# agussomacal/ROMHighContrast

Hardware: AMD Instinct MI355X
Metric: snapshot_solves_per_sec (higher is better)
Workload: dtype f64

## Files before the change

### romhighcontrast_amd/csrc/rom_fem_dev.h

```cpp
#pragma once
#include "rom_mma.h"

struct FemDev {
  int nrb, ncb, N, n1, n1p, nr, nc, nGp, nGa, T, nslots, kblk, npre, nrhs, nexp, ncross, xb0;
  long long dim;
  const double* pool;
  const int* alist;
  const int* aoff;
  int tile_stream;
  const int* pairs;
  int npairs;
  const double* pool_acc;
  const int* wmeta;
  int wp0[5];
  int s1_t0, s1_nterm, s1_ndr;
  const int* s1_items;
  const int* s1_citems;
  const GenTerm* terms;
  const double* Bt;
  const double* P;
  const double* vec;
  const RhsTerm* rhs;
  const PreEdge* pre;
  const ExpEdge* exp;
  const int* xred;
  const int* scb;
  int spos0, nsc, sblk0;
  const DenseGroup* dgroups;
  const int* dweight;
  const int* ditem_group;
  const int* ditem_k;
  const double* dmat;
  int ndg, ndi;
  const CoefGroup* groups;
  const double* cm;
  const int* item_group;
  const int* item_k;
  const int* item_cf;
  const int* ctask;
  int nctask, ncf;
  double* gdots;
  int ncoef;
  const double* G;
  const double* Gs;
  const double* A0;
  const double* Qp;
  const int* kmax;
  const int* epos;
  double* yhat;
  const double* W;
  const double* g;
  const TileDesc* desc;
  const int* kptr;
  const int* kpair;
  const int* colptr;
  const int* colrow;
  const int* colti;
  const BlockSide* sides;
  int n_lr;
  const int* lr_blocks;
  const int* gen_blocks;
  const int* vmap;
  const int* scat;
  int nscat;
  double* L;
  double* invL;
  double* y;
  int* status;
};


FemDev make_dev(const rom_fem* f);

constexpr int COEF_MAX = 64;
#ifndef PAIR_RING_
#define PAIR_RING_ 8
#endif
constexpr int PAIR_RING = PAIR_RING_;
constexpr int S1_COEF_BYTES = 4 * COEF_MAX * 8, S1_WAVE_BYTES = (40 * 64 + 64 * 4 + 64 + 64 + 3 * 64 * 4) * 8;
constexpr int S1_ITEM_PASSES = 4;
constexpr int S1_DENSE_BYTES = 64 * 64 * 8;
constexpr int S1_LDS_BYTES = S1_COEF_BYTES + 4 * S1_WAVE_BYTES + S1_DENSE_BYTES;
constexpr int DENSE_GROUPS_MAX = 8;

__host__ __device__ inline int h0_row(int s, int i, int j, int N, int n1) {
  int ii, jj;
  switch (s) {
    case 0: ii = i; jj = j; break;
    case 1: ii = N - i; jj = j; break;
    case 2: ii = j; jj = i; break;
    default: ii = N - j; jj = i; break;
  }
  return (ii - 1) * n1 + (jj - 1);
}

__global__ void k_repack_table(const double* __restrict__ G, int ld, int nseg, int n1, int orient, double* __restrict__ Gs);
__global__ void k_build_A0(double* A0, const double* Qp, const double* rho, int n1, int n1p, int N);
__global__ void k_rhs(FemDev f, const double* __restrict__ a);
__global__ void k_coef(FemDev f, const double* __restrict__ a);
__global__ void k_expand(FemDev f, const double* __restrict__ a, int Mc, double* __restrict__ U, long long row0);
__global__ void k_back_pre(FemDev f, const double* __restrict__ a, int Mc);
template <int NS>
__global__ void k_diag_update(FemDev f, const double* __restrict__ a, int slot, int Mc);
__global__ void k_diag_factor(FemDev f, int slot, int j);
__global__ void k_solve1(FemDev f, const double* __restrict__ a, int Mc);
template <int NS>
__global__ void k_factor_panel(FemDev f, const double* __restrict__ a, int j, int Mc);
__global__ void k_backsolve(FemDev f);
__global__ void k_edge_transform(FemDev f, int Mc);
__global__ void k_extend(FemDev f, const double* __restrict__ a, int Mc, double* __restrict__ U, long long row0, const int* __restrict__ blocks, int pw_log2);
constexpr int X128_BLOCKS = 16;
// ... 65 lines not shown
```

### romhighcontrast_amd/csrc/rom_fem_kernels.hip

```cpp
#include "rom_fem_dev.h"

__global__ void k_build_A0(double* A0, const double* Qp, const double* rho, int n1, int n1p, int N) {
  size_t idx = blockIdx.x * size_t(blockDim.x) + threadIdx.x;
  size_t total = size_t(n1) * n1 * n1p;
  if (idx >= total) return;
  int m = int(idx % n1p);
  size_t ij = idx / n1p;
  int j = int(ij % n1) + 1, i = int(ij / n1) + 1;
  A0[idx] = (m < n1) ? Qp[size_t(j - 1) * n1p + m] * rho[size_t(m) * (N + 1) + i] : 0.0;
}

__global__ void k_repack_table(const double* __restrict__ G, int ld, int nseg, int n1, int orient, double* __restrict__ Gs) {
  const long long idx = blockIdx.x * (long long)blockDim.x + threadIdx.x;
  const long long hrows = (long long)n1 * n1;
  if (idx >= (long long)nseg * hrows * 8) return;
  const int kk = int(idx & 7);
  const long long rp = (idx >> 3) % hrows, seg = (idx >> 3) / hrows;
  const long long row = orient ? (rp % n1) * n1 + rp / n1 : rp;
  const int k = int(seg) * 8 + kk;
  Gs[idx] = k < ld ? G[row * ld + k] : 0.0;
}


__device__ inline double readlane_f64(double v, int lane) {
// ... 1333 lines not shown
  for (int v = t; v < f.nGa; v += 256) ym[v] = xs[v];
}

__global__ __launch_bounds__(256) void k_edge_transform(FemDev f, int Mc) {
  __shared__ __align__(16) double lds[STAGE_TOTAL];
  const WavePos wp;
  const int pos = f.epos[blockIdx.z];
  const int srow = stage_row(), sseg = stage_seg();
  const int mA = blockIdx.y * 64 + srow;
  const double* pA = mA < Mc ? f.y + size_t(mA) * f.nGp + pos + sseg : nullptr;
  const double* pB = f.Qp + size_t(blockIdx.x * 64 + srow) * f.n1p + sseg;
  Acc acc;
  acc_zero(acc);
  gemm_loop(
      f.n1p / BK, [&](int ch, double* v) { load4_aligned(pA ? pA + ch * BK : nullptr, v); },
      [&](int ch, double* v) { load4_aligned(pB + ch * BK, v); }, acc, lds, wp);
#pragma unroll
  for (int i = 0; i < 2; ++i)
#pragma unroll
    for (int g = 0; g < 4; ++g) {
      const int m = blockIdx.y * 64 + acc_row(wp, i, g);
      if (m >= Mc) continue;
#pragma unroll
      for (int jb = 0; jb < 2; ++jb)
        f.yhat[size_t(m) * f.nGp + pos + blockIdx.x * 64 + acc_col(wp, jb)] = acc.c[i][jb][g];
    }
}


__global__ __launch_bounds__(256) void k_extend(FemDev f, const double* __restrict__ a, int Mc,
                                                double* __restrict__ U, long long row0, const int* __restrict__ blocks,
                                                int pw_log2) {
  __shared__ __align__(16) double lds[STAGE_TOTAL];
  __shared__ double scs[64];
  double* stage = lds;
  const WavePos wp;
  const int b = blocks[blockIdx.z];
  const int p = b / f.ncb, q = b % f.ncb;
  const int n1 = f.n1, N = f.N;
  const BlockSide& sd = f.sides[b];
  const int srow = stage_row(), sseg = stage_seg();
  const int pw = 1 << pw_log2, ph = 64 >> pw_log2;
  const int npj = (n1 + pw - 1) >> pw_log2;
  const int pi = blockIdx.x / npj, pj = blockIdx.x % npj;
  const int i0 = ph * pi + 1, j0 = pw * pj + 1;
  const int i1 = min(i0 + ph - 1, n1), j1 = min(j0 + pw - 1, n1);

  const int mA = blockIdx.y * 64 + srow;
  const bool vA = mA < Mc;
  const int iB = i0 + (srow >> pw_log2), jB = j0 + (srow & (pw - 1));
  const bool vB = iB <= n1 && jB <= n1;

  int cend[4];
  const double* pAs[4];
  const double* pBs[4];
  int tot = 0;
#pragma unroll
  for (int s = 0; s < 4; ++s) {
    const ExtSide es = sd.s[s];
    int nch = 0;
    pAs[s] = pBs[s] = nullptr;
    if (es.mode != 0) {
      const int hrow = vB ? h0_row(s, iB, jB, N, n1) : 0;
      if (es.mode == 1) {
        const int dist = s == 0 ? i0 : s == 1 ? N - i1 : s == 2 ? j0 : N - j1;
        nch = f.kmax[dist] / BK;
        if (vA) pAs[s] = f.yhat + size_t(mA) * f.nGp + es.off + sseg;
        if (vB) pBs[s] = f.A0 + size_t(hrow) * f.n1p + sseg;
      } else {
        nch = es.nch;
        if (vA) pAs[s] = f.y + size_t(mA) * f.nGp + es.off + sseg;
        if (vB) pBs[s] = f.G + es.gtab + size_t(hrow) * (es.nch * BK) + sseg;
      }
    }
    tot += nch;
    cend[s] = tot;
  }
  if (threadIdx.x < 64) {
    const int m = blockIdx.y * 64 + threadIdx.x;
    scs[threadIdx.x] = m < Mc ? f.y[size_t(m) * f.nGp + f.sblk0 + b] : 0.0;
  }
  __syncthreads();
  Acc acc;
  acc_zero(acc);
  auto pick = [&](int ch, const double* const* ps) -> const double* {
    const int s = (ch >= cend[0]) + (ch >= cend[1]) + (ch >= cend[2]);
    const int lc = ch - (s == 0 ? 0 : s == 1 ? cend[0] : s == 2 ? cend[1] : cend[2]);
    const double* p = s == 0 ? ps[0] : s == 1 ? ps[1] : s == 2 ? ps[2] : ps[3];
    return p ? p + lc * BK : nullptr;
  };
  gemm_loop(
      tot, [&](int ch, double* v) { load4_aligned(pick(ch, pAs), v); },
      [&](int ch, double* v) { load4_aligned(pick(ch, pBs), v); }, acc, stage, wp);

  const bool odd = wp.lane & 1;
  const int cfirst = acc_col(wp, odd ? 1 : 0) - (odd ? 1 : 0);
  const int ii = i0 + (cfirst >> pw_log2) - 1, jj = j0 + (cfirst & (pw - 1)) - 1;
  const bool v0 = ii < n1 && jj < n1, v1 = ii < n1 && jj + 1 < n1;
  const long long gidx = (long long)(p * N + ii) * f.nc + (q * N + jj);
  double w_own[2];
#pragma unroll
  for (int jb = 0; jb < 2; ++jb) {
    const int cidx = acc_col(wp, jb);
    const int wi = i0 + (cidx >> pw_log2) - 1, wj = j0 + (cidx & (pw - 1)) - 1;
    w_own[jb] = (wi < n1 && wj < n1) ? f.W[wi * n1 + wj] : 0.0;
  }
#pragma unroll
  for (int i = 0; i < 2; ++i)
#pragma unroll
    for (int g = 0; g < 4; ++g) {
      const int m = blockIdx.y * 64 + acc_row(wp, i, g);
      const double sc = scs[acc_row(wp, i, g)];
      const double x0 = acc.c[i][0][g] + sc * w_own[0], x1 = acc.c[i][1][g] + sc * w_own[1];
      const double got = lane_swap1(odd ? x0 : x1);
      if (m >= Mc) continue;
      double* dst = U + (row0 + m) * f.dim + gidx;
      const double lo = odd ? got : x0, hi = odd ? x1 : got;
      if (v1) *reinterpret_cast<double2_u*>(dst) = double2_u{lo, hi};
      else if (v0) dst[0] = lo;
    }
}



constexpr int X128_SLOT = 4 * 128 * 64;

template <bool FLAT>
__global__ __launch_bounds__(512, 2) void k_extend128(FemDev f, X128Args xa, const double* __restrict__ a, int Mc,
                                                      double* __restrict__ U, long long row0, int with_expand,
                                                      int sys_fast) {
  __shared__ __align__(16) char lds_bytes[2 * X128_SLOT];
  __shared__ double scs[128];
  double* const lds = reinterpret_cast<double*>(lds_bytes);
  const int n1 = f.n1, N = f.N;
  const int nct = (n1 + 127) / 128;
  const int nvert = n1 * n1;
  const int ntile = FLAT ? (nvert + 127) / 128 : n1 * nct;
  int bx, by, ngy;
  if (sys_fast > 0) {
    bx = int(blockIdx.x) / sys_fast; by = int(blockIdx.x) % sys_fast; ngy = sys_fast;
  } else if (sys_fast < 0) {
    ngy = -sys_fast;
    const int unit = int(blockIdx.x) / (8 * ngy), r = int(blockIdx.x) % (8 * ngy);
    bx = unit * 8 + (r & 7); by = r >> 3;
  } else {
    bx = int(blockIdx.x); by = int(blockIdx.y); ngy = int(gridDim.y);
  }
  if (bx >= ntile + with_expand) return;
  if (bx >= ntile) {
    static_assert(STAGE_TOTAL * sizeof(double) <= 2 * X128_SLOT, "expansion staging must fit");
    const int nx = f.n1p / 64, ny = (Mc + 63) / 64;
    const int item = (bx - ntile) + with_expand * (by + ngy * blockIdx.z);
    if (threadIdx.x >= 256) return;
    if (item < nx * ny * (f.nexp + 1)) expand_tile(f, Mc, U, row0, lds, item % nx, (item / nx) % ny, item / (nx * ny));
    return;
  }
  const int bz = blockIdx.z;
  {
    const unsigned lin = __builtin_amdgcn_readfirstlane(blockIdx.x + gridDim.x * (blockIdx.y + gridDim.y * bz));
    if (lin >= 256u && lin < 512u)
      for (int i = 0; i < 2; ++i) __builtin_amdgcn_s_sleep(127);
  }
  const int b = xa.blocks[bz];
  const int p = b / f.ncb, q = b % f.ncb;
  const BlockSide sd = xa.sides[bz];
  const int iv = bx / nct + 1;
  const int jv0 = 128 * (bx % nct) + 1;
  const int vt0 = 128 * bx;
  const int lane = threadIdx.x & 63, w = __builtin_amdgcn_readfirstlane(threadIdx.x >> 6), wr = w >> 2, wc = w & 3;
  constexpr int NJ = 2;
  const int fr = lane & 15, kq = lane >> 4;
  double my_sc = 0.0;
  if (threadIdx.x < 128) {
    const int m = by * 128 + threadIdx.x;
    if (m < Mc) my_sc = f.y[size_t(m) * f.nGp + f.sblk0 + b];
  }
  double w_own[NJ];
#pragma unroll
  for (int j = 0; j < NJ; ++j) {
    if (FLAT) {
      const int v = vt0 + wc * (16 * NJ) + j * 16 + fr;
      w_own[j] = v < nvert ? f.W[v] : 0.0;
    } else {
      const int jj = jv0 + wc * (16 * NJ) + j * 16 + fr;
      w_own[j] = jj <= n1 ? f.W[(iv - 1) * n1 + (jj - 1)] : 0.0;
    }
  }
  const int cnt0 = sd.s[0].mode == 2 ? min(2 * sd.s[0].nch, (sd.s[0].r + 1 + 7) / 8) : 0;
  const int cnt1 = sd.s[1].mode == 2 ? min(2 * sd.s[1].nch, (sd.s[1].r + 1 + 7) / 8) : 0;
  const int cnt2 = sd.s[2].mode == 2 ? min(2 * sd.s[2].nch, (sd.s[2].r + 1 + 7) / 8) : 0;
  const int cnt3 = sd.s[3].mode == 2 ? min(2 * sd.s[3].nch, (sd.s[3].r + 1 + 7) / 8) : 0;
  const int nseg = cnt0 + cnt1 + cnt2 + cnt3;
  const int tot = (nseg + 1) / 2;
  const unsigned fx = unsigned((kq >> 1) ^ (fr >> 2));
  const unsigned fa0 = unsigned(fr * 64) + (fx << 4) + unsigned(kq & 1) * 8u;
  const unsigned fa1 = unsigned(fr * 64) + ((fx ^ 2u) << 4) + unsigned(kq & 1) * 8u;
#define X_FRAGS(SLOT_, KKI_, AF_, BF_)                                                                             \
  do {                                                                                                             \
    const char* pf_ = lds_bytes + (SLOT_) * X128_SLOT + (((KKI_)&1) ? fa1 : fa0);                                  \
    const char* pa_ = pf_ + ((KKI_) >> 1) * 8192 + wr * 4096;                                                      \
    const char* pb_ = pf_ + 16384 + ((KKI_) >> 1) * 8192 + wc * (1024 * NJ);                                       \
    _Pragma("unroll") for (int i_ = 0; i_ < 4; ++i_) AF_[i_] = *reinterpret_cast<const double*>(pa_ + i_ * 1024);  \
    _Pragma("unroll") for (int i_ = 0; i_ < NJ; ++i_) BF_[i_] = *reinterpret_cast<const double*>(pb_ + i_ * 1024); \
  } while (0)
  const unsigned lds0 = unsigned(size_t((__attribute__((address_space(3))) char*)lds_bytes));
  const unsigned du16 = unsigned(((lane & 3) ^ ((lane >> 4) & 3)) * 16);
  const unsigned ybytes_row = unsigned(f.nGp) * 8u;
  const int m0 = by * 128;
  unsigned voA[2];
  int vi[2], vj[2];
#pragma unroll
  for (int g = 0; g < 2; ++g) {
    const int rl = 32 * (w & 3) + 16 * g + (lane >> 2);
    voA[g] = unsigned(max(0, min(rl, Mc - 1 - m0))) * ybytes_row + du16;
    if (FLAT) {
      const int v = min(vt0 + rl, nvert - 1);
      vi[g] = v / n1 + 1;
      vj[g] = v % n1 + 1;
    } else {
      vi[g] = iv;
      vj[g] = min(jv0 + rl, n1);
    }
  }
  const char* const ybase = reinterpret_cast<const char*>(f.y) + size_t(min(m0, Mc - 1)) * ybytes_row;
  const char* const gsbase = reinterpret_cast<const char*>(f.Gs);
  const size_t seg_stride = size_t(n1) * n1 * 64;
  const char* const zbase = reinterpret_cast<const char*>(f.W + size_t(n1) * n1);
  const unsigned voZ = unsigned(lane) * 16u;
  int c_side = -1, c_left = 0, c_segs = nseg;
  const char* pA = zbase;
  const char* pB = zbase;
  unsigned voB[2] = {0, 0};
#define X_NEXT_SIDE()                                                                                              \
  do {                                                                                                             \
    do {                                                                                                           \
      ++c_side;                                                                                                    \
      c_left = c_side == 0 ? cnt0 : c_side == 1 ? cnt1 : c_side == 2 ? cnt2 : cnt3;                                \
    } while (c_left == 0 && c_side < 3);                                                                           \
    const int off_ = c_side == 0 ? sd.s[0].off : c_side == 1 ? sd.s[1].off : c_side == 2 ? sd.s[2].off : sd.s[3].off; \
    const int gseg_ = c_side == 0 ? sd.s[0].gseg : c_side == 1 ? sd.s[1].gseg : c_side == 2 ? sd.s[2].gseg : sd.s[3].gseg; \
     \
         \
    const int ci_ = c_side == 1 ? -n1 : n1, cj_ = c_side == 3 ? -1 : 1;                                             \
    const int k0_ = c_side == 1 ? n1 * n1 - 1 : c_side == 3 ? -n1 + n1 : -n1 - 1;                                   \
    pA = ybase + size_t(off_) * 8;                                                                                 \
    pB = gsbase + size_t(gseg_) * 8;                                                                               \
    voB[0] = unsigned(ci_ * vi[0] + cj_ * vj[0] + k0_) * 64u + du16;                                               \
    voB[1] = unsigned(ci_ * vi[1] + cj_ * vj[1] + k0_) * 64u + du16;                                               \
  } while (0)
#define X_DMA(LDS_, BASE_, VOFF_)                                                                                  \
  asm volatile("s_mov_b32 m0, %0\n\tglobal_load_lds_dwordx4 %1, %2" ::"s"(__builtin_amdgcn_readfirstlane(LDS_)),   \
               "v"(VOFF_), "s"(x128_uniform(BASE_))                                                                \
               : "memory", "m0")
#define X_ISSUE_HALF(SLOT_, H_, MINE_)                                                                             \
  do {                                                                                                             \
    const unsigned sb_ = lds0 + unsigned(SLOT_) * X128_SLOT + (H_) * 8192 + unsigned(w & 3) * 2048;                \
    if (c_segs > 0) {                                                                                              \
      if (MINE_) {                                                                                                 \
        X_DMA(sb_, pA, voA[0]);                                                                                    \
        X_DMA(sb_ + 1024, pA, voA[1]);                                                                             \
        X_DMA(sb_ + 16384, pB, voB[0]);                                                                            \
        X_DMA(sb_ + 16384 + 1024, pB, voB[1]);                                                                     \
      }                                                                                                            \
      pA += 64;                                                                                                    \
      pB += seg_stride;                                               \
      --c_segs;                                                                                                    \
      if (--c_left == 0 && c_segs > 0) X_NEXT_SIDE();                                                              \
    } else if (MINE_) {                                                 \
      X_DMA(sb_, zbase, voZ);                                                                                      \
      X_DMA(sb_ + 1024, zbase, voZ);                                                                               \
      X_DMA(sb_ + 16384, zbase, voZ);                                                                              \
      X_DMA(sb_ + 16384 + 1024, zbase, voZ);                                                                       \
    }                                                                                                              \
  } while (0)
  d4_t acc[4][NJ];
#pragma unroll
  for (int i = 0; i < 4; ++i)
#pragma unroll
    for (int j = 0; j < NJ; ++j) acc[i][j] = d4_t{0.0, 0.0, 0.0, 0.0};
  if (tot > 0) {
    X_NEXT_SIDE();
    X_ISSUE_HALF(0, 0, w < 4);
    X_ISSUE_HALF(0, 1, w < 4);
    asm volatile("s_waitcnt vmcnt(0)\n\ts_barrier" ::: "memory");
    double af[2][4], bf[2][NJ];
    X_FRAGS(0, 0, af[0], bf[0]);
    for (int ch = 0; ch < tot; ++ch) {
      const int slot = ch & 1;
      if (ch + 1 < tot) {
        const bool mine = (w >> 2) == ((ch + 1) & 1);
        X_ISSUE_HALF(slot ^ 1, 0, mine);
        X_ISSUE_HALF(slot ^ 1, 1, mine);
      }
#pragma unroll
      for (int kki = 0; kki < 4; ++kki) {
        const int pb = kki & 1;
        if (kki < 3) X_FRAGS(slot, kki + 1, af[pb ^ 1], bf[pb ^ 1]);
#pragma unroll
        for (int i = 0; i < 4; ++i)
#pragma unroll
          for (int j = 0; j < NJ; ++j) acc[i][j] = __builtin_amdgcn_mfma_f64_16x16x4f64(af[pb][i], bf[pb][j], acc[i][j], 0, 0, 0);
      }
      {
        asm volatile("s_waitcnt vmcnt(0)\n\ts_barrier" ::: "memory");
      }
      if (ch + 1 < tot) X_FRAGS(slot ^ 1, 0, af[0], bf[0]);
    }
  }
#undef X_ISSUE_HALF
#undef X_DMA
#undef X_NEXT_SIDE
#undef X_FRAGS
#ifndef ROMHC_EPI_PRIO
#define ROMHC_EPI_PRIO 3
#endif
#ifndef X128_STORE_POLICY
#define X128_STORE_POLICY ""
#endif
  __builtin_amdgcn_s_setprio(ROMHC_EPI_PRIO);
  if (threadIdx.x < 128) scs[threadIdx.x] = my_sc;
  __syncthreads();
  const bool odd = lane & 1;
  constexpr int NHP = NJ / 2;
  char* sp[NHP];
  long long d1[NHP] = {};
  unsigned long long k16[NHP], k8[NHP], k8b[NHP];
  {
    char* const rowp = reinterpret_cast<char*>(U) + size_t(row0 + m0 + wr * 64 + kq) * size_t(f.dim) * 8;
#pragma unroll
    for (int hp = 0; hp < NHP; ++hp) {
      const int t = wc * (16 * NJ) + (2 * hp + (odd ? 1 : 0)) * 16 + fr - (odd ? 1 : 0);
      long long off0, off1;
      bool ok0, ok1;
      if (FLAT) {
        const int v = vt0 + t, i0 = v / n1, j0 = v - i0 * n1;
        off0 = (long long)(p * N + i0) * f.nc + q * N + j0;
        off1 = j0 + 1 < n1 ? off0 + 1 : (long long)(p * N + i0 + 1) * f.nc + q * N;
        ok0 = v < nvert;
        ok1 = v + 1 < nvert;
      } else {
        const int jcol = jv0 + t;
        off0 = (long long)(p * N + iv - 1) * f.nc + q * N - 1 + jcol;
        off1 = off0 + 1;
        ok0 = jcol <= n1;
        ok1 = jcol + 1 <= n1;
      }
      const bool straddle = FLAT && off1 != off0 + 1;
      k16[hp] = __builtin_amdgcn_ballot_w64(ok1 && !straddle);
      k8[hp] = __builtin_amdgcn_ballot_w64(ok0 && (!ok1 || straddle));
      k8b[hp] = __builtin_amdgcn_ballot_w64(ok1 && straddle);
      sp[hp] = rowp + off0 * 8;
      d1[hp] = (off1 - off0) * 8;
    }
  }
  const long long step = 4ll * f.dim * 8;
  const bool full = m0 + 128 <= Mc;
  const int mrow = m0 + wr * 64 + kq;
#pragma unroll
  for (int i = 0; i < 4; ++i)
#pragma unroll
    for (int g = 0; g < 4; ++g) {
      const double sc = scs[wr * 64 + i * 16 + kq + 4 * g];
// ... 55 lines not shown
```

### romhighcontrast_amd/csrc/rom_fem_setup.hip

```cpp
#include <algorithm>
#include <array>
#include <cmath>
#include <cstdlib>
#include <cstring>
#include <map>
#include <atomic>
#include <set>
#include <thread>

#include <chrono>
#include <tuple>

#include "rom_fem_dev.h"
#include "rom_hostla.h"

#ifdef ROMHC_AB
static const char* ab_env(const char* name) { return getenv(name); }
#else
static const char* ab_env(const char*) { return nullptr; }
#endif

FemDev make_dev(const rom_fem* f) {
  FemDev d;
  d.nrb = f->nrb; d.ncb = f->ncb; d.N = f->N; d.n1 = f->n1; d.n1p = f->n1p; d.nr = f->nr; d.nc = f->nc;
  d.nGp = f->nGp; d.nGa = f->nGa; d.npre = f->npre; d.nrhs = f->nrhs; d.nexp = f->nexp; d.ncross = f->ncross;
  d.xb0 = f->xb0; d.pool = f->d_pool; d.alist = f->d_alist; d.aoff = f->d_aoff; d.tile_stream = f->sw_no_tile_stream ? 0 : 1; d.pairs = f->d_pairs; d.npairs = f->npairs; d.pool_acc = f->d_pool_acc; d.wmeta = f->d_wmeta; d.s1_items = f->d_s1_items; d.s1_citems = f->d_s1_citems; for (int i = 0; i < 5; ++i) d.wp0[i] = f->wp0[i]; d.s1_t0 = d.s1_nterm = d.s1_ndr = 0; if (f->fused1 && !f->desc.empty()) { d.s1_t0 = f->desc[0].t0; d.s1_nterm = f->desc[0].t1 - f->desc[0].t0; d.s1_ndr = f->desc[0].ndr; } d.terms = f->d_terms; d.Bt = f->d_Bt; d.P = f->d_P; d.vec = f->d_vec;
  d.rhs = f->d_rhs; d.pre = f->d_pre; d.exp = f->d_exp; d.xred = f->d_xred; d.scb = f->d_scb; d.spos0 = f->spos0; d.nsc = f->nsc;
  d.sblk0 = f->spos0 + f->n_all_edges; d.groups = f->d_groups; d.cm = f->d_cm; d.item_group = f->d_item_group;
  d.item_k = f->d_item_k; d.item_cf = f->d_item_cf; d.ctask = f->d_ctask; d.nctask = f->nctask; d.ncf = f->ncf; d.ncoef = f->ncoef; d.dgroups = f->d_dgroups; d.dweight = f->d_dweight;
  d.ditem_group = f->d_ditem_group; d.ditem_k = f->d_ditem_k; d.dmat = f->d_dmat; d.ndg = f->ndg; d.ndi = f->ndi; d.T = f->T; d.nslots = f->nslots;
  d.kblk = f->nrb * f->ncb; d.dim = f->dim;
  d.G = f->d_G; d.Gs = f->d_Gs; d.A0 = f->d_A0; d.Qp = f->d_Qp; d.kmax = f->d_kmax; d.epos = f->d_epos; d.yhat = f->d_yhat; d.W = f->d_W;
  d.g = f->d_g; d.desc = f->d_desc;
  d.kptr = f->d_kptr; d.kpair = f->d_kpair; d.colptr = f->d_colptr; d.colrow = f->d_colrow;
  d.colti = f->d_colti; d.sides = f->d_sides; d.lr_blocks = f->d_lr_blocks; d.n_lr = f->n_lr_blocks; d.gen_blocks = f->d_gen_blocks; d.vmap = f->d_vmap; d.scat = f->d_scat; d.nscat = f->nscat; d.L = f->d_L; d.invL = f->d_invL;
  d.y = f->d_y; d.status = f->ctx->d_status; d.gdots = f->d_dots;
  return d;
}

namespace {

using hostla::ld;
using hostla::Mat;

struct Edge {
  int hv, p, q;
  int b0, b1;
};

struct Small {
  int rpos, cpos;
  Mat tab;
  int kind;
  std::array<int, 4> b;
};

struct Comp {
  int r = 0;
  Mat W;
  Mat Kt;
  Mat P;
  std::vector<ld> gt;
  std::vector<ld> p0;
  Mat KiW;
  std::vector<ld> wK;
};

template <class F>
void parallel_for(size_t n, F fn) {
  const unsigned nthr = std::max(1u, std::min<unsigned>(std::thread::hardware_concurrency(), unsigned(n)));
  std::atomic<size_t> next{0};
  auto work = [&]() {
    for (size_t i = next++; i < n; i = next++) fn(i);
  };
  std::vector<std::thread> pool;
  for (unsigned t = 1; t < nthr; ++t) pool.emplace_back(work);
  work();
  for (auto& th : pool) th.join();
}

struct UnitBlock {
  int N, n1;
  Mat Q, rho;
  std::vector<ld> lam, kappa;
  Mat Wl;
  Mat Kmat, Kinv;
  std::vector<ld> gE[2];
  std::vector<double> rho_d, Wd;

// ... 284 lines not shown
    std::vector<char> busy(nrb * ncb, 0);
    for (int e = 0; e < E; ++e)
      if (!busy[edges[e].b0] && !busy[edges[e].b1]) { is_pre[e] = 1; busy[edges[e].b0] = busy[edges[e].b1] = 1; }
  }
  std::vector<int> pre_list, pre_index(E, -1);
  for (int e = 0; e < E; ++e)
    if (is_pre[e]) { pre_index[e] = int(pre_list.size()); pre_list.push_back(e); }
  const int npre = int(pre_list.size());
  const int nact = E - npre;

  ROMHC_PHASE("elimination order of the active edges (greedy mi");
  std::vector<int> order, ord_of(E, -1);
  {
    std::vector<std::set<int>> g(E);
    for (int e = 0; e < E; ++e)
      if (!is_pre[e])
        for (int x : adj[e])
          if (!is_pre[x]) g[e].insert(x);
    for (int e : pre_list)
      for (int x : adj[e])
        for (int y : adj[e])
          if (x != y && !is_pre[x] && !is_pre[y]) g[x].insert(y);
    std::vector<char> done(E, 0);
    for (int step = 0; step < nact; ++step) {
      int best = -1;
      size_t bd = 0;
      for (int e = 0; e < E; ++e) {
        if (done[e] || is_pre[e]) continue;
        if (best < 0 || g[e].size() < bd) { best = e; bd = g[e].size(); }
      }
      done[best] = 1;
      ord_of[best] = int(order.size());
      order.push_back(best);
      std::vector<int> nb(g[best].begin(), g[best].end());
      for (int x : nb) {
        g[x].erase(best);
        for (int y : nb)
          if (x != y) g[x].insert(y);
      }
    }
  }

  ROMHC_PHASE("unit-block tables in long double, compression of");
  UnitBlock ub(N, E > 0);
  const Mat& Q = ub.Q;
  const Mat& Kinv = ub.Kinv;
  const std::vector<ld>* gE = ub.gE;
  const std::vector<double>& rho_d = ub.rho_d;
  const std::vector<double>& Wd = ub.Wd;
  const double h2 = 1.0 / (double(N) * double(N));
  auto Tm = [&](int id) -> const Mat& { return ub.Tm(id); };
  auto TK = [&](int id) -> const Mat& { return ub.TK(id); };
  const bool compress = !getenv("ROMHC_NO_COMPRESS");
  ld ctol = 1e-14L;
  if (const char* s = getenv("ROMHC_COMPRESS_TOL")) ctol = (ld)atof(s);
  const ld ckeep = std::min<ld>(ctol, 1e-17L);
  std::map<std::vector<int>, int> sig_id;
  std::vector<std::vector<int>> sigs;
  std::vector<int> comp_of(E, -1);
  for (int e = 0; e < E; ++e) {
    const Edge& ed = edges[e];
    std::vector<int> sig{ed.hv};
    for (int blk : {ed.b0, ed.b1}) {
      const int sf = side_of(blk, e);
      for (int s2 = 0; s2 < 4; ++s2)
        if (s2 != sf && bside[blk][s2] >= 0) sig.push_back(sf * 4 + s2);
    }
    bool x0 = false, x1 = false;
    for (auto& c : xc)
      if (c.edge == e) (c.node == 0 ? x0 : x1) = true;
    sig.push_back(100 + (x0 ? 1 : 0) + (x1 ? 2 : 0));
    auto it = sig_id.find(sig);
    if (it == sig_id.end()) {
      it = sig_id.emplace(sig, int(sigs.size())).first;
      sigs.push_back(sig);
    }
    comp_of[e] = it->second;
  }
  std::vector<Comp> comps(sigs.size());
  {
    std::vector<int> ids, ids_tk;
    for (auto& sig : sigs)
      for (size_t t = 1; t + 1 < sig.size(); ++t) ids.push_back(sig[t]);
    for (int e : pre_list)
      for (int u : adj[e]) {
        const int blk = shared_block(e, u);
        ids_tk.push_back(side_of(blk, u) * 4 + side_of(blk, e));
        ids.push_back(side_of(blk, e) * 4 + side_of(blk, u));
      }
    ub.prepare(ids, false);
    ub.prepare(ids_tk, true);
    std::vector<char> ok(sigs.size(), 1);
    std::vector<Mat> Wfull(sigs.size());
    std::vector<std::vector<ld>> pivots(sigs.size());
    if (compress)
      parallel_for(sigs.size(), [&](size_t c) {
        const std::vector<int>& sig = sigs[c];
        const int flags = sig.back() - 100;
        compress_basis(ub, std::vector<int>(sig.begin() + 1, sig.end() - 1), flags & 1, flags & 2, ckeep, Wfull[c], pivots[c]);
      });
    std::vector<int> r_drop(sigs.size(), n1), r_use(sigs.size(), n1);
    if (compress) {
      std::vector<int> r_fill(sigs.size(), n1);
      for (size_t c = 0; c < sigs.size(); ++c) {
        int r = 0;
        while (r < int(pivots[c].size()) && pivots[c][r] > ctol * pivots[c][0]) ++r;
        r_drop[c] = r;
        r_fill[c] = std::min<int>(int(pivots[c].size()), (r + 1 + 7) / 8 * 8 - 1);
      }
      auto tiles = [&](const std::vector<int>& rr) {
        long long nred_ = ncross;
        for (int e : order) nred_ += std::min(rr[comp_of[e]], n1);
        return (nred_ + TB - 1) / TB;
      };
      r_use = tiles(r_fill) <= tiles(r_drop) ? r_fill : r_drop;
    }
    parallel_for(sigs.size(), [&](size_t c) {
      ok[c] = compress_finish(ub, Wfull[c], r_use[c], sigs[c][0], compress, comps[c]);
    });
    for (char o : ok)
      if (!o) { rom_set_error("internal: compressed edge block not positive definite"); return ROM_ERR_INVALID; }
  }

  std::vector<int> kmax(N + 1, n1p);
  double kavg = 0;
  for (int dd = 1; dd <= N; ++dd) {
    int last = -1;
    for (int m = 0; m < n1; ++m)
      if (rho_d[size_t(m) * (N + 1) + std::min(dd, N)] >= 1e-18) last = m;
    kmax[dd] = std::min(n1p, std::max(BK, (last + 1 + BK - 1) / BK * BK));
    if (dd <= n1) kavg += kmax[dd] / double(std::max(n1, 1));
  }
  kmax[0] = n1p;
  std::vector<int> rp(comps.size(), 0);
  std::vector<char> use_lr(comps.size(), 0);
  for (size_t c = 0; c < comps.size(); ++c) {
    rp[c] = (comps[c].r + 1 + BK - 1) / BK * BK;
    use_lr[c] = comps[c].r < n1 && rp[c] <= 1.25 * kavg && n1 > 0 && !getenv("ROMHC_NO_LOWRANK_EXT");
  }

  ROMHC_PHASE("layout of the reduced vector: edge groups in eli");
  std::vector<int> zpos(E, -1), rk(E, 0), xred(ncross, -1), xhost(ncross, -1);
  for (int x = 0; x < ncross; ++x)
    for (auto& c : xc)
      if (c.cross == x && !is_pre[c.edge] && (xhost[x] < 0 || ord_of[c.edge] > ord_of[xhost[x]])) xhost[x] = c.edge;
  int nred = 0;
  {
    int total = ncross;
    for (int e : order) total += comps[comp_of[e]].r;
    if (total <= TB)
      for (int x = 0; x < ncross; ++x) xred[x] = nred++;
  }
  for (int e : order) {
    zpos[e] = nred;
    rk[e] = comps[comp_of[e]].r;
    nred += rk[e];
    f->ranks.push_back(rk[e]);
    for (int x = 0; x < ncross; ++x)
      if (xhost[x] == e && xred[x] < 0) xred[x] = nred++;
  }
  for (int x = 0; x < ncross; ++x)
// ... 846 lines not shown
```

### romhighcontrast_amd/csrc/rom_mma.h

```cpp
#pragma once
#include <hip/hip_runtime.h>

#include "romhc_internal.h"

typedef double d4_t __attribute__((ext_vector_type(4)));

struct Acc {
  d4_t c[2][2];
};

__device__ inline void acc_zero(Acc& a) {
#pragma unroll
  for (int i = 0; i < 2; ++i)
#pragma unroll
    for (int j = 0; j < 2; ++j) a.c[i][j] = d4_t{0.0, 0.0, 0.0, 0.0};
}

constexpr int STAGE_DOUBLES = 64 * LDK;
constexpr int STAGE_TOTAL = 4 * STAGE_DOUBLES;
constexpr int TILE_DOUBLES = 64 * LDC;

struct WavePos {
  int lane, wr, wc;
  __device__ WavePos() {
    lane = threadIdx.x & 63;
    int w = threadIdx.x >> 6;
    wr = w >> 1;
    wc = w & 1;
  }
};

__device__ inline int acc_row(const WavePos& wp, int i, int g) { return wp.wr * 32 + i * 16 + (wp.lane >> 4) + 4 * g; }
__device__ inline int acc_col(const WavePos& wp, int j) { return wp.wc * 32 + j * 16 + (wp.lane & 15); }

__device__ inline void mma_chunk(const double* __restrict__ sA, const double* __restrict__ sB, Acc& acc,
                                 const WavePos& wp) {
  const int r = wp.lane & 15, kq = wp.lane >> 4;
  const double* pa = sA + (wp.wr * 32 + r) * LDK + kq;
  const double* pb = sB + (wp.wc * 32 + r) * LDK + kq;
#pragma unroll
  for (int kk = 0; kk < BK; kk += 4) {
    double a0 = pa[kk], a1 = pa[16 * LDK + kk];
    double b0 = pb[kk], b1 = pb[16 * LDK + kk];
    acc.c[0][0] = __builtin_amdgcn_mfma_f64_16x16x4f64(a0, b0, acc.c[0][0], 0, 0, 0);
    acc.c[0][1] = __builtin_amdgcn_mfma_f64_16x16x4f64(a0, b1, acc.c[0][1], 0, 0, 0);
    acc.c[1][0] = __builtin_amdgcn_mfma_f64_16x16x4f64(a1, b0, acc.c[1][0], 0, 0, 0);
    acc.c[1][1] = __builtin_amdgcn_mfma_f64_16x16x4f64(a1, b1, acc.c[1][1], 0, 0, 0);
  }
}

__device__ inline void mma_chunk_Atile(const double* __restrict__ tileA, int k0, const double* __restrict__ sB,
                                       Acc& acc, const WavePos& wp) {
  const int r = wp.lane & 15, kq = wp.lane >> 4;
  const double* pa = tileA + (wp.wr * 32 + r) * LDC + k0 + kq;
  const double* pb = sB + (wp.wc * 32 + r) * LDK + kq;
#pragma unroll
  for (int kk = 0; kk < BK; kk += 4) {
    double a0 = pa[kk], a1 = pa[16 * LDC + kk];
    double b0 = pb[kk], b1 = pb[16 * LDK + kk];
    acc.c[0][0] = __builtin_amdgcn_mfma_f64_16x16x4f64(a0, b0, acc.c[0][0], 0, 0, 0);
    acc.c[0][1] = __builtin_amdgcn_mfma_f64_16x16x4f64(a0, b1, acc.c[0][1], 0, 0, 0);
    acc.c[1][0] = __builtin_amdgcn_mfma_f64_16x16x4f64(a1, b0, acc.c[1][0], 0, 0, 0);
    acc.c[1][1] = __builtin_amdgcn_mfma_f64_16x16x4f64(a1, b1, acc.c[1][1], 0, 0, 0);
  }
}

__device__ inline int stage_row() { return threadIdx.x >> 2; }
__device__ inline int stage_seg() { return (threadIdx.x & 3) * 4; }

__device__ inline void stage_store(double* s, const double v[4]) {
  double* p = s + stage_row() * LDK + stage_seg();
  *reinterpret_cast<double2*>(p) = double2{v[0], v[1]};
  *reinterpret_cast<double2*>(p + 2) = double2{v[2], v[3]};
}

__device__ inline void load4_aligned(const double* __restrict__ p, double v[4]) {
  if (p) {
    double2 x = *reinterpret_cast<const double2*>(p);
    double2 y = *reinterpret_cast<const double2*>(p + 2);
    v[0] = x.x; v[1] = x.y; v[2] = y.x; v[3] = y.y;
  } else {
    v[0] = v[1] = v[2] = v[3] = 0.0;
  }
}

template <class FA, class FB, class FP>
__device__ inline void gemm_loop2(int nchunks, FA loadA, FB loadB, FP active, Acc& acc, double* stA, double* stB,
                                  const WavePos& wp) {
  if (nchunks <= 0) return;
  double va[4], vb[4];
  loadA(0, va);
  loadB(0, vb);
  for (int ch = 0; ch < nchunks; ++ch) {
    double* sA = stA + (ch & 1) * STAGE_DOUBLES;
    double* sB = stB + (ch & 1) * STAGE_DOUBLES;
    stage_store(sA, va);
    stage_store(sB, vb);
    __syncthreads();
    if (ch + 1 < nchunks) {
      loadA(ch + 1, va);
      loadB(ch + 1, vb);
    }
    if (active(ch)) mma_chunk(sA, sB, acc, wp);
  }
  __syncthreads();
}

__device__ inline int kmajor_k() { return threadIdx.x & 15; }
__device__ inline int kmajor_row(int x) { return (threadIdx.x >> 4) + 16 * x; }
__device__ inline void stage_store_kmajor(double* s, const double v[4]) {
#pragma unroll
  for (int x = 0; x < 4; ++x) s[kmajor_row(x) * LDK + kmajor_k()] = v[x];
}

template <class FA, class FB>
__device__ inline void gemm_loop_kmajor(int nchunks, FA loadA, FB loadB, Acc& acc, double* stage, const WavePos& wp) {
  if (nchunks <= 0) return;
  double va[4], vb[4];
  loadA(0, va);
  loadB(0, vb);
  for (int ch = 0; ch < nchunks; ++ch) {
    double* sA = stage + (ch & 1) * STAGE_DOUBLES;
    double* sB = stage + 2 * STAGE_DOUBLES + (ch & 1) * STAGE_DOUBLES;
    stage_store_kmajor(sA, va);
    stage_store_kmajor(sB, vb);
    __syncthreads();
    if (ch + 1 < nchunks) {
      loadA(ch + 1, va);
      loadB(ch + 1, vb);
    }
    mma_chunk(sA, sB, acc, wp);
  }
  __syncthreads();
}

template <class FA, class FB>
__device__ inline void gemm_loop(int nchunks, FA loadA, FB loadB, Acc& acc, double* stage, const WavePos& wp) {
  gemm_loop2(nchunks, loadA, loadB, [](int) { return true; }, acc, stage, stage + 2 * STAGE_DOUBLES, wp);
}

template <class FB, class FP>
__device__ inline void gemm_loop_Atile(const double* tileA, int nchunks, FB loadB, FP active, Acc& acc, double* stB,
                                       const WavePos& wp) {
  double vb[4];
  loadB(0, vb);
  for (int ch = 0; ch < nchunks; ++ch) {
    double* sB = stB + (ch & 1) * STAGE_DOUBLES;
    stage_store(sB, vb);
    __syncthreads();
    if (ch + 1 < nchunks) loadB(ch + 1, vb);
    if (active(ch)) mma_chunk_Atile(tileA, ch * BK, sB, acc, wp);
  }
  __syncthreads();
}
```

### romhighcontrast_amd/csrc/romhc_internal.h

```cpp
#pragma once
#include <hip/hip_runtime.h>

#include <cstdarg>
#include <cstdint>
#include <cstdio>
#include <map>
#include <string>
#include <vector>

#include "romhc.h"

void rom_set_error(const char* fmt, ...);

#define ROM_HIP(call)                                                                      \
  do {                                                                                     \
    hipError_t _e = (call);                                                                \
    if (_e != hipSuccess) {                                                                \
      rom_set_error("%s failed: %s (%s:%d)", #call, hipGetErrorString(_e), __FILE__, __LINE__); \
      return ROM_ERR_HIP;                                                                  \
    }                                                                                      \
  } while (0)

#define ROM_CHECK(cond, ...)      \
  do {                            \
// ... 157 lines not shown
  int nexp;
  int ncross, xb0;
  int T;
  int nslots;
  double* d_G = nullptr;
  double* d_Gs = nullptr;
  double* d_A0 = nullptr;
  double* d_Qp = nullptr;
  int* d_kmax = nullptr;
  int* d_epos = nullptr;
  int n_edges = 0;
  double ext_flops = 0;
  double* d_yhat = nullptr;
  double* d_dots = nullptr;
  double* d_W = nullptr;
  double* d_g = nullptr;
  TileDesc* d_desc = nullptr;
  GenTerm* d_terms = nullptr;
  double* d_pool = nullptr;
  int* d_pairs = nullptr;
  int* d_alist = nullptr;
  int* d_aoff = nullptr;
  int npairs = 0;
  double* d_pool_acc = nullptr;
  int* d_wmeta = nullptr;
  int wp0[5] = {};
  int* d_s1_items = nullptr;
  int* d_s1_citems = nullptr;
  int* d_kptr = nullptr;
  int* d_kpair = nullptr;
  int* d_colptr = nullptr;
  int* d_colrow = nullptr;
  int* d_colti = nullptr;
  double* d_Bt = nullptr;
  double* d_P = nullptr;
  double* d_vec = nullptr;
  RhsTerm* d_rhs = nullptr;
  PreEdge* d_pre = nullptr;
  ExpEdge* d_exp = nullptr;
  int* d_xred = nullptr;
  int* d_scb = nullptr;
  int spos0 = 0, nsc = 0, n_all_edges = 0;
  CoefGroup* d_groups = nullptr;
  double* d_cm = nullptr;
  int* d_item_group = nullptr;
  int* d_item_k = nullptr;
  int ncoef = 0;
  int* d_item_cf = nullptr;
  int* d_ctask = nullptr;
  int nctask = 0, ncf = 0;
  bool lds_optin_coef = false;
  bool fused1 = false;
  bool sw_no_fused = false, sw_no_ext128 = false, sw_no_fold = false;
  int sw_x128_sys_fast = -1;
  size_t gs_bytes = 0;
  int sw_ext_flat = -1;
  bool sw_coef_global = false;
  bool sw_no_tile_pairs = false;
  bool sw_no_tile_stream = false;
  DenseGroup* d_dgroups = nullptr;
  int* d_dweight = nullptr;
  int* d_ditem_group = nullptr;
  int* d_ditem_k = nullptr;
  double* d_dmat = nullptr;
  int ndg = 0, ndi = 0;
  int nrhs = 0;
  BlockSide* d_sides = nullptr;
  int* d_lr_blocks = nullptr;
  std::vector<int> lr_blocks_host;
  int* d_gen_blocks = nullptr;
  int n_lr_blocks = 0, n_gen_blocks = 0, lr_nch = 0;
  int* d_vmap = nullptr;
  int* d_scat = nullptr;
  int nscat = 0;
  std::vector<TileDesc> desc;
  std::vector<int> slot_of, kptr, kpair, colptr, colrow, colti, diag_slot;
  std::vector<BlockSide> sides;
  std::vector<int> ranks;
  double flops_solve = 0, bytes_solve = 0;
  void* fmap = nullptr;
  double* d_riesz = nullptr;
  double* d_green = nullptr;
  double* d_L = nullptr;
  double* d_invL = nullptr;
  double* d_y = nullptr;
  int ws_M = 0;
};

int rom_launch_gemm_nt(rom_ctx* ctx, int64_t m, int64_t n, int64_t k, double alpha, const double* A,
                       int64_t lda, const double* B, int64_t ldb, double beta, double* C, int64_t ldc,
                       const char* prof_name);
int rom_launch_gemm_nt_ex(rom_ctx* ctx, int64_t m, int64_t n, int64_t k, double alpha, const double* A,
                          int64_t lda, const double* B, int64_t ldb, double beta, double* C, int64_t ldc,
                          const char* prof_name, int lower_only);

void rom_factored_map_free(void* map);
int rom_launch_pack_reduced(rom_fem* f, const double* Y, double* Yc, int M, hipStream_t st);
```

Before: 4.165 million.

## Trim extension GEMM K-loop to actual compressed rank at 4-wide granularity

```diff
diff --git a/romhighcontrast_amd/csrc/rom_fem_dev.h b/romhighcontrast_amd/csrc/rom_fem_dev.h
--- a/romhighcontrast_amd/csrc/rom_fem_dev.h
+++ b/romhighcontrast_amd/csrc/rom_fem_dev.h
@@ -57,6 +57,7 @@
   const int* colrow;
   const int* colti;
   const BlockSide* sides;
+  int ext_full_k;
   int n_lr;
   const int* lr_blocks;
   const int* gen_blocks;
diff --git a/romhighcontrast_amd/csrc/rom_fem_kernels.hip b/romhighcontrast_amd/csrc/rom_fem_kernels.hip
--- a/romhighcontrast_amd/csrc/rom_fem_kernels.hip
+++ b/romhighcontrast_amd/csrc/rom_fem_kernels.hip
@@ -1409,6 +1409,7 @@
   const bool vB = iB <= n1 && jB <= n1;
 
   int cend[4];
+  int klast[4];
   const double* pAs[4];
   const double* pBs[4];
   int tot = 0;
@@ -1416,6 +1417,7 @@
   for (int s = 0; s < 4; ++s) {
     const ExtSide es = sd.s[s];
     int nch = 0;
+    klast[s] = BK / 4;
     pAs[s] = pBs[s] = nullptr;
     if (es.mode != 0) {
       const int hrow = vB ? h0_row(s, iB, jB, N, n1) : 0;
@@ -1426,6 +1428,7 @@
         if (vB) pBs[s] = f.A0 + size_t(hrow) * f.n1p + sseg;
       } else {
         nch = es.nch;
+        if (!f.ext_full_k) klast[s] = min(BK / 4, max(1, (es.r + 1 - BK * (es.nch - 1) + 3) / 4));
         if (vA) pAs[s] = f.y + size_t(mA) * f.nGp + es.off + sseg;
         if (vB) pBs[s] = f.G + es.gtab + size_t(hrow) * (es.nch * BK) + sseg;
       }
@@ -1446,9 +1449,12 @@
     const double* p = s == 0 ? ps[0] : s == 1 ? ps[1] : s == 2 ? ps[2] : ps[3];
     return p ? p + lc * BK : nullptr;
   };
-  gemm_loop(
+  auto ksteps = [&](int ch) {
+    return ch + 1 == cend[0] ? klast[0] : ch + 1 == cend[1] ? klast[1] : ch + 1 == cend[2] ? klast[2] : ch + 1 == cend[3] ? klast[3] : BK / 4;
+  };
+  gemm_loop_ksteps(
       tot, [&](int ch, double* v) { load4_aligned(pick(ch, pAs), v); },
-      [&](int ch, double* v) { load4_aligned(pick(ch, pBs), v); }, acc, stage, wp);
+      [&](int ch, double* v) { load4_aligned(pick(ch, pBs), v); }, ksteps, acc, stage, stage + 2 * STAGE_DOUBLES, wp);
 
   const bool odd = wp.lane & 1;
   const int cfirst = acc_col(wp, odd ? 1 : 0) - (odd ? 1 : 0);
@@ -1543,12 +1549,17 @@
       w_own[j] = jj <= n1 ? f.W[(iv - 1) * n1 + (jj - 1)] : 0.0;
     }
   }
-  const int cnt0 = sd.s[0].mode == 2 ? min(2 * sd.s[0].nch, (sd.s[0].r + 1 + 7) / 8) : 0;
-  const int cnt1 = sd.s[1].mode == 2 ? min(2 * sd.s[1].nch, (sd.s[1].r + 1 + 7) / 8) : 0;
-  const int cnt2 = sd.s[2].mode == 2 ? min(2 * sd.s[2].nch, (sd.s[2].r + 1 + 7) / 8) : 0;
-  const int cnt3 = sd.s[3].mode == 2 ? min(2 * sd.s[3].nch, (sd.s[3].r + 1 + 7) / 8) : 0;
+  const int full_k = f.ext_full_k;
+#define X_UNITS(S_) (sd.s[S_].mode == 2 ? min(4 * sd.s[S_].nch, full_k ? (sd.s[S_].r + 1 + 7) / 8 * 2 : (sd.s[S_].r + 1 + 3) / 4) : 0)
+  const int un0 = X_UNITS(0), un1 = X_UNITS(1), un2 = X_UNITS(2), un3 = X_UNITS(3);
+#undef X_UNITS
+  const int cnt0 = (un0 + 1) >> 1, cnt1 = (un1 + 1) >> 1, cnt2 = (un2 + 1) >> 1, cnt3 = (un3 + 1) >> 1;
   const int nseg = cnt0 + cnt1 + cnt2 + cnt3;
   const int tot = (nseg + 1) / 2;
+#ifndef X128_HALF_SEG_LOADS
+#define X128_HALF_SEG_LOADS 1
+#endif
+  const unsigned long long lm_half = __builtin_amdgcn_ballot_w64((((lane & 3) ^ ((lane >> 4) & 3)) & 2) == 0);
   const unsigned fx = unsigned((kq >> 1) ^ (fr >> 2));
   const unsigned fa0 = unsigned(fr * 64) + (fx << 4) + unsigned(kq & 1) * 8u;
   const unsigned fa1 = unsigned(fr * 64) + ((fx ^ 2u) << 4) + unsigned(kq & 1) * 8u;
@@ -1584,7 +1595,8 @@
   const size_t seg_stride = size_t(n1) * n1 * 64;
   const char* const zbase = reinterpret_cast<const char*>(f.W + size_t(n1) * n1);
   const unsigned voZ = unsigned(lane) * 16u;
-  int c_side = -1, c_left = 0, c_segs = nseg;
+  int c_side = -1, c_left = 0, c_segs = nseg, c_odd = 0;
+  unsigned n_mask = 0;
   const char* pA = zbase;
   const char* pB = zbase;
   unsigned voB[2] = {0, 0};
@@ -1593,6 +1605,7 @@
     do {                                                                                                           \
       ++c_side;                                                                                                    \
       c_left = c_side == 0 ? cnt0 : c_side == 1 ? cnt1 : c_side == 2 ? cnt2 : cnt3;                                \
+      c_odd = (c_side == 0 ? un0 : c_side == 1 ? un1 : c_side == 2 ? un2 : un3) & 1;                               \
     } while (c_left == 0 && c_side < 3);                                                                           \
     const int off_ = c_side == 0 ? sd.s[0].off : c_side == 1 ? sd.s[1].off : c_side == 2 ? sd.s[2].off : sd.s[3].off; \
     const int gseg_ = c_side == 0 ? sd.s[0].gseg : c_side == 1 ? sd.s[1].gseg : c_side == 2 ? sd.s[2].gseg : sd.s[3].gseg; \
@@ -1609,25 +1622,46 @@
   asm volatile("s_mov_b32 m0, %0\n\tglobal_load_lds_dwordx4 %1, %2" ::"s"(__builtin_amdgcn_readfirstlane(LDS_)),   \
                "v"(VOFF_), "s"(x128_uniform(BASE_))                                                                \
                : "memory", "m0")
+#define X_DMA_LANES(LDS_, BASE_, VOFF_, LM_)                                                                       \
+  do {                                                                                                             \
+    unsigned long long sv_;                                                                                        \
+    asm volatile("s_mov_b64 %0, exec\n\ts_mov_b64 exec, %1\n\ts_mov_b32 m0, %2\n\tglobal_load_lds_dwordx4 %3, %4\n\t" \
+                 "s_mov_b64 exec, %0"                                                                              \
+                 : "=&s"(sv_)                                                                                      \
+                 : "s"(LM_), "s"(__builtin_amdgcn_readfirstlane(LDS_)), "v"(VOFF_), "s"(x128_uniform(BASE_))       \
+                 : "memory", "m0");                                                                                \
+  } while (0)
 #define X_ISSUE_HALF(SLOT_, H_, MINE_)                                                                             \
   do {                                                                                                             \
     const unsigned sb_ = lds0 + unsigned(SLOT_) * X128_SLOT + (H_) * 8192 + unsigned(w & 3) * 2048;                \
     if (c_segs > 0) {                                                                                              \
+      const bool half_ = c_left == 1 && c_odd != 0;         \
+      n_mask |= (half_ ? 1u : 3u) << (2 * (H_));                                                                   \
       if (MINE_) {                                                                                                 \
-        X_DMA(sb_, pA, voA[0]);                                                                                    \
-        X_DMA(sb_ + 1024, pA, voA[1]);                                                                             \
-        X_DMA(sb_ + 16384, pB, voB[0]);                                                                            \
-        X_DMA(sb_ + 16384 + 1024, pB, voB[1]);                                                                     \
+        if (half_ && X128_HALF_SEG_LOADS) {                                                                        \
+          X_DMA_LANES(sb_, pA, voA[0], lm_half);                                                                   \
+          X_DMA_LANES(sb_ + 1024, pA, voA[1], lm_half);                                                            \
+          X_DMA_LANES(sb_ + 16384, pB, voB[0], lm_half);                                                           \
+          X_DMA_LANES(sb_ + 16384 + 1024, pB, voB[1], lm_half);                                                    \
+        } else {                                                                                                   \
+          X_DMA(sb_, pA, voA[0]);                                                                                  \
+          X_DMA(sb_ + 1024, pA, voA[1]);                                                                           \
+          X_DMA(sb_ + 16384, pB, voB[0]);                                                                          \
+          X_DMA(sb_ + 16384 + 1024, pB, voB[1]);                                                                   \
+        }                                                                                                          \
       }                                                                                                            \
       pA += 64;                                                                                                    \
       pB += seg_stride;                                               \
       --c_segs;                                                                                                    \
       if (--c_left == 0 && c_segs > 0) X_NEXT_SIDE();                                                              \
-    } else if (MINE_) {                                                 \
-      X_DMA(sb_, zbase, voZ);                                                                                      \
-      X_DMA(sb_ + 1024, zbase, voZ);                                                                               \
-      X_DMA(sb_ + 16384, zbase, voZ);                                                                              \
-      X_DMA(sb_ + 16384 + 1024, zbase, voZ);                                                                       \
+    } else if (full_k) {  \
+      n_mask |= 3u << (2 * (H_));                                                                                  \
+      if (MINE_) {                                                                                                 \
+        X_DMA(sb_, zbase, voZ);                                                                                    \
+        X_DMA(sb_ + 1024, zbase, voZ);                                                                             \
+        X_DMA(sb_ + 16384, zbase, voZ);                                                                            \
+        X_DMA(sb_ + 16384 + 1024, zbase, voZ);                                                                     \
+      }                                                                                                            \
     }                                                                                                              \
   } while (0)
   d4_t acc[4][NJ];
@@ -1644,6 +1678,8 @@
     X_FRAGS(0, 0, af[0], bf[0]);
     for (int ch = 0; ch < tot; ++ch) {
       const int slot = ch & 1;
+      const unsigned k_mask = __builtin_amdgcn_readfirstlane(n_mask);
+      n_mask = 0;
       if (ch + 1 < tot) {
         const bool mine = (w >> 2) == ((ch + 1) & 1);
         X_ISSUE_HALF(slot ^ 1, 0, mine);
@@ -1652,11 +1688,13 @@
 #pragma unroll
       for (int kki = 0; kki < 4; ++kki) {
         const int pb = kki & 1;
-        if (kki < 3) X_FRAGS(slot, kki + 1, af[pb ^ 1], bf[pb ^ 1]);
-#pragma unroll
-        for (int i = 0; i < 4; ++i)
-#pragma unroll
-          for (int j = 0; j < NJ; ++j) acc[i][j] = __builtin_amdgcn_mfma_f64_16x16x4f64(af[pb][i], bf[pb][j], acc[i][j], 0, 0, 0);
+        if (kki < 3 && (k_mask >> (kki + 1) & 1u)) X_FRAGS(slot, kki + 1, af[pb ^ 1], bf[pb ^ 1]);
+        if (k_mask >> kki & 1u) {
+#pragma unroll
+          for (int i = 0; i < 4; ++i)
+#pragma unroll
+            for (int j = 0; j < NJ; ++j) acc[i][j] = __builtin_amdgcn_mfma_f64_16x16x4f64(af[pb][i], bf[pb][j], acc[i][j], 0, 0, 0);
+        }
       }
       {
         asm volatile("s_waitcnt vmcnt(0)\n\ts_barrier" ::: "memory");
@@ -1665,6 +1703,7 @@
     }
   }
 #undef X_ISSUE_HALF
+#undef X_DMA_LANES
 #undef X_DMA
 #undef X_NEXT_SIDE
 #undef X_FRAGS
diff --git a/romhighcontrast_amd/csrc/rom_fem_setup.hip b/romhighcontrast_amd/csrc/rom_fem_setup.hip
--- a/romhighcontrast_amd/csrc/rom_fem_setup.hip
+++ b/romhighcontrast_amd/csrc/rom_fem_setup.hip
@@ -34,7 +34,7 @@
   d.g = f->d_g; d.desc = f->d_desc;
   d.kptr = f->d_kptr; d.kpair = f->d_kpair; d.colptr = f->d_colptr; d.colrow = f->d_colrow;
   d.colti = f->d_colti; d.sides = f->d_sides; d.lr_blocks = f->d_lr_blocks; d.n_lr = f->n_lr_blocks; d.gen_blocks = f->d_gen_blocks; d.vmap = f->d_vmap; d.scat = f->d_scat; d.nscat = f->nscat; d.L = f->d_L; d.invL = f->d_invL;
-  d.y = f->d_y; d.status = f->ctx->d_status; d.gdots = f->d_dots;
+  d.y = f->d_y; d.status = f->ctx->d_status; d.gdots = f->d_dots; d.ext_full_k = f->sw_ext_full_k ? 1 : 0;
   return d;
 }
 
@@ -425,6 +425,8 @@
   auto Tm = [&](int id) -> const Mat& { return ub.Tm(id); };
   auto TK = [&](int id) -> const Mat& { return ub.TK(id); };
   const bool compress = !getenv("ROMHC_NO_COMPRESS");
+  const int kgran = getenv("ROMHC_K_GRANULE") && atoi(getenv("ROMHC_K_GRANULE")) == 8 ? 8 : 4;
+  f->sw_ext_full_k = kgran == 8 || (getenv("ROMHC_EXT_FULL_K") && atoi(getenv("ROMHC_EXT_FULL_K")) != 0);
   ld ctol = 1e-14L;
   if (const char* s = getenv("ROMHC_COMPRESS_TOL")) ctol = (ld)atof(s);
   const ld ckeep = std::min<ld>(ctol, 1e-17L);
@@ -479,7 +481,7 @@
         int r = 0;
         while (r < int(pivots[c].size()) && pivots[c][r] > ctol * pivots[c][0]) ++r;
         r_drop[c] = r;
-        r_fill[c] = std::min<int>(int(pivots[c].size()), (r + 1 + 7) / 8 * 8 - 1);
+        r_fill[c] = std::min<int>(int(pivots[c].size()), (r + 1 + kgran - 1) / kgran * kgran - 1);
       }
       auto tiles = [&](const std::vector<int>& rr) {
         long long nred_ = ncross;
diff --git a/romhighcontrast_amd/csrc/rom_mma.h b/romhighcontrast_amd/csrc/rom_mma.h
--- a/romhighcontrast_amd/csrc/rom_mma.h
+++ b/romhighcontrast_amd/csrc/rom_mma.h
@@ -33,19 +33,34 @@
 __device__ inline int acc_row(const WavePos& wp, int i, int g) { return wp.wr * 32 + i * 16 + (wp.lane >> 4) + 4 * g; }
 __device__ inline int acc_col(const WavePos& wp, int j) { return wp.wc * 32 + j * 16 + (wp.lane & 15); }
 
+__device__ inline void mma_kstep(const double* __restrict__ pa, const double* __restrict__ pb, int kk, Acc& acc) {
+  double a0 = pa[kk], a1 = pa[16 * LDK + kk];
+  double b0 = pb[kk], b1 = pb[16 * LDK + kk];
+  acc.c[0][0] = __builtin_amdgcn_mfma_f64_16x16x4f64(a0, b0, acc.c[0][0], 0, 0, 0);
+  acc.c[0][1] = __builtin_amdgcn_mfma_f64_16x16x4f64(a0, b1, acc.c[0][1], 0, 0, 0);
+  acc.c[1][0] = __builtin_amdgcn_mfma_f64_16x16x4f64(a1, b0, acc.c[1][0], 0, 0, 0);
+  acc.c[1][1] = __builtin_amdgcn_mfma_f64_16x16x4f64(a1, b1, acc.c[1][1], 0, 0, 0);
+}
+
 __device__ inline void mma_chunk(const double* __restrict__ sA, const double* __restrict__ sB, Acc& acc,
                                  const WavePos& wp) {
   const int r = wp.lane & 15, kq = wp.lane >> 4;
   const double* pa = sA + (wp.wr * 32 + r) * LDK + kq;
   const double* pb = sB + (wp.wc * 32 + r) * LDK + kq;
 #pragma unroll
-  for (int kk = 0; kk < BK; kk += 4) {
-    double a0 = pa[kk], a1 = pa[16 * LDK + kk];
-    double b0 = pb[kk], b1 = pb[16 * LDK + kk];
-    acc.c[0][0] = __builtin_amdgcn_mfma_f64_16x16x4f64(a0, b0, acc.c[0][0], 0, 0, 0);
-    acc.c[0][1] = __builtin_amdgcn_mfma_f64_16x16x4f64(a0, b1, acc.c[0][1], 0, 0, 0);
-    acc.c[1][0] = __builtin_amdgcn_mfma_f64_16x16x4f64(a1, b0, acc.c[1][0], 0, 0, 0);
-    acc.c[1][1] = __builtin_amdgcn_mfma_f64_16x16x4f64(a1, b1, acc.c[1][1], 0, 0, 0);
+  for (int kk = 0; kk < BK; kk += 4) mma_kstep(pa, pb, kk, acc);
+}
+
+__device__ inline void mma_chunk(const double* __restrict__ sA, const double* __restrict__ sB, Acc& acc,
+                                 const WavePos& wp, int nk) {
+  if (nk >= BK / 4) {
+    mma_chunk(sA, sB, acc, wp);
+  } else if (nk > 0) {
+    nk = __builtin_amdgcn_readfirstlane(nk);
+    const int r = wp.lane & 15, kq = wp.lane >> 4;
+    const double* pa = sA + (wp.wr * 32 + r) * LDK + kq;
+    const double* pb = sB + (wp.wc * 32 + r) * LDK + kq;
+    for (int k = 0; k < nk; ++k) mma_kstep(pa, pb, 4 * k, acc);
   }
 }
 
@@ -84,9 +99,9 @@
   }
 }
 
-template <class FA, class FB, class FP>
-__device__ inline void gemm_loop2(int nchunks, FA loadA, FB loadB, FP active, Acc& acc, double* stA, double* stB,
-                                  const WavePos& wp) {
+template <class FA, class FB, class FK>
+__device__ inline void gemm_loop_ksteps(int nchunks, FA loadA, FB loadB, FK ksteps, Acc& acc, double* stA, double* stB,
+                                        const WavePos& wp) {
   if (nchunks <= 0) return;
   double va[4], vb[4];
   loadA(0, va);
@@ -101,9 +116,15 @@
       loadA(ch + 1, va);
       loadB(ch + 1, vb);
     }
-    if (active(ch)) mma_chunk(sA, sB, acc, wp);
+    mma_chunk(sA, sB, acc, wp, ksteps(ch));
   }
   __syncthreads();
+}
+
+template <class FA, class FB, class FP>
+__device__ inline void gemm_loop2(int nchunks, FA loadA, FB loadB, FP active, Acc& acc, double* stA, double* stB,
+                                  const WavePos& wp) {
+  gemm_loop_ksteps(nchunks, loadA, loadB, [&](int ch) { return active(ch) ? BK / 4 : 0; }, acc, stA, stB, wp);
 }
 
 __device__ inline int kmajor_k() { return threadIdx.x & 15; }
diff --git a/romhighcontrast_amd/csrc/romhc_internal.h b/romhighcontrast_amd/csrc/romhc_internal.h
--- a/romhighcontrast_amd/csrc/romhc_internal.h
+++ b/romhighcontrast_amd/csrc/romhc_internal.h
@@ -233,6 +233,7 @@
   bool lds_optin_coef = false;
   bool fused1 = false;
   bool sw_no_fused = false, sw_no_ext128 = false, sw_no_fold = false;
+  bool sw_ext_full_k = false;
   int sw_x128_sys_fast = -1;
   size_t gs_bytes = 0;
   int sw_ext_flat = -1;
```

Measured after the change: 4.417 million (median of 6 runs). 1.06x the previous value.
